# sedaprotocol/bn254

Measured on AMD Instinct MI355X. Metric: BN254 pairings/sec (batch verify), higher is better.
Workload: dtype u32

## Files before the change

bn254_amd/csrc/bn254_field.h:

```cpp
#pragma once
#include <stdint.h>

#if defined(__HIPCC__)
#include <hip/hip_runtime.h>
#define BN_DEV __device__ __forceinline__
#define BN_DEVN __device__ __noinline__
#define BN_CONST __device__ __constant__ const
#if defined(BN_INLINE_FP12_HOT)
#define BN_DEVH BN_DEV
#else
#define BN_DEVH BN_DEVN
#endif
#if defined(BN_INLINE_FE_HOT)
#define BN_DEVF BN_DEV
#else
#define BN_DEVF BN_DEVN
#endif
#if defined(__HIP_DEVICE_COMPILE__) && !defined(BN_NO_ASSUME_LDS)
#define BN_ASSUME_LDS(ptr) __builtin_assume(__builtin_amdgcn_is_shared((const void*)(ptr)))
#else
#define BN_ASSUME_LDS(ptr) do { } while (0)
#endif
#if defined(BN_INLINE_MILLER)
#define BN_DEVM BN_DEV
// ... 1052 lines not shown
  fp6_inv(d, d);
  fp6_mul<91>(t0, a.c1, d);
  fp6_mul<95>(r.c0, a.c0, d);
  fp6_neg(r.c1, t0);
}
#if defined(BN_INLINE_MUL_LINE)
BN_DEVH void fp12_mul_line(Fp12& r, const Fp12& f, const Fp2& l0, const Fp2& l1, const Fp2& l2) {
#else
BN_DEVN void fp12_mul_line(Fp12& r, const Fp12& f, const Fp2& l0, const Fp2& l1, const Fp2& l2) {
#endif
  Fp6 t0, t1, s, u;
  fp6_mul_fp2(t0, f.c0, l0);
  fp6_mul_01<110>(t1, f.c1, l1, l2);
  fp6_add(s, f.c0, f.c1); fp6_site_n<113>(s, s);
  fp6_mul_01<116>(u, s, NS(119, fp2_add(l0, l1)), l2);
  fp6_sub(u, u, t0);
  fp6_sub(u, u, t1);
  fp6_mul_v(s, t1);
  fp6_add(s, t0, s);
  fp6_site_r<120>(r.c0, s);
  fp6_site_r<123>(r.c1, u);
}
#if defined(BN_SPLIT_FP2) && defined(BN_FP6_LAZY) && !defined(BN_FP6_LAZY_ONLY_SQR)
BN_DEVH void fp12_mul_line2(Fp12& r, const Fp12& f, const Fp6& b0, const Fp2& b10, const Fp2& b11) {
  Fp6 t0, t1, s, u, bs;
  fp6_mul_lazy(t0, f.c0, b0);
  fp6_mul_01_lazy(t1, f.c1, b10, b11);
  fp6_add(s, f.c0, f.c1);
  bs.c0 = NS(306, fp2_add(b0.c0, b10)); bs.c1 = NS(307, fp2_add(b0.c1, b11)); bs.c2 = b0.c2;
  fp6_mul_lazy(u, s, bs);
  fp6_sub(u, u, t0);
  fp6_sub(u, u, t1);
  fp6_mul_v(s, t1);
  fp6_add(s, t0, s);
  fp6_site_r<308>(r.c0, s);
  fp6_site_r<311>(r.c1, u);
}
#else
BN_DEVH void fp12_mul_line2(Fp12& r, const Fp12& f, const Fp6& b0, const Fp2& b10, const Fp2& b11) {
  Fp6 t0, t1, s, u, bs;
  fp6_mul<140>(t0, f.c0, b0);
  fp6_mul_01<144>(t1, f.c1, b10, b11);
  fp6_add(s, f.c0, f.c1); fp6_site_n<147>(s, s);
  bs.c0 = NS(150, fp2_add(b0.c0, b10)); bs.c1 = NS(151, fp2_add(b0.c1, b11)); bs.c2 = b0.c2;
  fp6_mul<152>(u, s, bs);
  fp6_sub(u, u, t0);
  fp6_sub(u, u, t1);
  fp6_mul_v(s, t1);
  fp6_add(s, t0, s);
  fp6_site_r<156>(r.c0, s);
  fp6_site_r<159>(r.c1, u);
}
#endif
BN_DEV Fp2& fp12_coef(Fp12& a, int k) {
  Fp6& h = (k & 1) ? a.c1 : a.c0;
  return (k >> 1) == 0 ? h.c0 : (k >> 1) == 1 ? h.c1 : h.c2;
}
BN_DEV void fp12_frob_body(Fp12& r, const Fp12& a, int power) {
  Fp12 t = a;
  for (int k = 0; k < 6; ++k) {
    Fp2& c = fp12_coef(t, k);
    Fp2 x = (power & 1) ? fp2_conj(c) : c;
    const int32_t (*g)[BN_LIMBS] = power == 1 ? C_FROB1[k] : power == 2 ? C_FROB2[k] : C_FROB3[k];
    c = fp2_mul(x, fp2_load_const(g));
  }
  r = t;
}
BN_DEVN void fp12_frob(Fp12& r, const Fp12& a, int power) { fp12_frob_body(r, a, power); }
template <int S> BN_DEV void fp4_sqr(Fp2& r0, Fp2& r1, const Fp2& a, const Fp2& b) {
  Fp2 a2 = fp2_sqr(a), b2 = fp2_sqr(b);
  r1 = NS(S + 1, fp2_sub(fp2_sub(fp2_sqr(NS(S, fp2_add(a, b))), a2), b2));
  r0 = NS(S + 2, fp2_add(a2, fp2_mul_xi(b2)));
}
template <int S> BN_DEV void fp12_cyclotomic_sqr_body(Fp12& r, const Fp12& a) {
#if defined(BN_TRIO_DEVICE)
  const int g = trio_g3();
  Fp2 x, y, ae, ao, e, o;
#pragma unroll
  for (int i = 0; i < BN_LIMBS; ++i) {
    x.c[0].v[i] = g == 0 ? a.c0.c0.c[0].v[i] : g == 1 ? a.c1.c0.c[0].v[i] : a.c0.c1.c[0].v[i];
    y.c[0].v[i] = g == 0 ? a.c1.c1.c[0].v[i] : g == 1 ? a.c0.c2.c[0].v[i] : a.c1.c2.c[0].v[i];
    ae.c[0].v[i] = g == 0 ? a.c0.c0.c[0].v[i] : g == 1 ? a.c0.c1.c[0].v[i] : a.c0.c2.c[0].v[i];
    ao.c[0].v[i] = g == 0 ? a.c1.c1.c[0].v[i] : g == 1 ? a.c1.c2.c[0].v[i] : a.c1.c0.c[0].v[i];
  }
  fp4_sqr<S + 20>(e, o, x, y);
  const Fp2 oxi = NS(S + 9, fp2_mul_xi(o));
#pragma unroll
  for (int i = 0; i < BN_LIMBS; ++i) o.c[0].v[i] = g == 2 ? oxi.c[0].v[i] : o.c[0].v[i];
  e = fp2_lin2_reduce(e, 3, ae, -2);
  o = fp2_lin2_reduce(o, 3, ao, 2);
  const unsigned base = BN_TRIO_X6_OFF + (threadIdx.x >> 3) * BN_TRIO_X6_STRIDE, mine = base + (threadIdx.x & 7u) * (3 * BN_LIMBS);
  BN_TRIO_FENCE();
#pragma unroll
  for (int i = 0; i < BN_LIMBS; ++i) { bn_trio_lds[mine + i] = e.c[0].v[i]; bn_trio_lds[mine + BN_LIMBS + i] = o.c[0].v[i]; }
  BN_TRIO_FENCE();
  const unsigned role = threadIdx.x & 1u;
  Fp12 out;
  Fp2* dst[6] = {&out.c0.c0, &out.c1.c1, &out.c0.c1, &out.c1.c2, &out.c0.c2, &out.c1.c0};
#pragma unroll
  for (int k = 0; k < 3; ++k) {
    const unsigned from = base + (2 * k + role) * (3 * BN_LIMBS);
#pragma unroll
    for (int i = 0; i < BN_LIMBS; ++i) { dst[2 * k]->c[0].v[i] = bn_trio_lds[from + i]; dst[2 * k + 1]->c[0].v[i] = bn_trio_lds[from + BN_LIMBS + i]; }
  }
  BN_TRIO_FENCE();
  r = out;
// ... 21 lines not shown
```

bn254_amd/csrc/bn254_hip.hip:

```cpp
#include <hip/hip_runtime.h>
#include <thread>

#include <cstdio>
#include <cstdlib>
#include <cstring>
#include <new>

#include "../../include/bn254_hip.h"
#include "bn254_hash.h"
#include "bn254_io.h"
#include "bn254_pairing.h"

using namespace bn254;

#include "bn254_ws.h"
#include "bn254_lane.h"
#include "bn254_host.h"

KERNEL_SMALL void k_decode_g1(const uint8_t* pts, size_t n, uint32_t flags, Ws ws, int px, int inf_plane, int accumulate) {
  size_t i = (size_t)blockIdx.x * BN_WAVE + threadIdx.x;
  if (i >= n) return;
  G1Affine p;
  uint8_t st = decode_g1(p, pts + 64 * i, flags);
  if (st != ST_OK) g1_set_generator(p);
// ... 814 lines not shown
  if (option == BN254_OPT_TRIO_WAVE_ROLES) {
    if (value < 0 || value > 2 || (value == 2 && !c->fits_w8) || (value == 1 && !c->fits_quad)) return BN254_E_BAD_ARGUMENT;
    c->trio_wave_roles = value;
    return 0;
  }
  if (option == BN254_OPT_HASH_DIRECT_WIDTH) {
    if (value < 0 || value > 32 || (value & (value - 1))) return BN254_E_BAD_ARGUMENT;
    c->hash_direct_width = value;
    return 0;
  }
  if (option == BN254_OPT_HASH_SCHEDULE) { if (value < 0 || value > 2) return BN254_E_BAD_ARGUMENT; c->hash_schedule = value; return 0; }
  if (option == BN254_OPT_HASH_WIDE_WIDTH) { if (value < 0 || value > 64) return BN254_E_BAD_ARGUMENT; c->hash_wide_width = value; return 0; }
  if (option == BN254_OPT_HASH_TAIL_CHUNK) {
    if (value < 2 || value > 32 || (value & (value - 1))) return BN254_E_BAD_ARGUMENT;
    c->hash_tail_chunk = value;
    return 0;
  }
  if (option == BN254_OPT_NONET_MAX_BATCH) {
    HIP_TRY(hipSetDevice(c->device));
    if (value < 0 || (value > 0 && !bn254_nonet_fits_device())) return BN254_E_BAD_ARGUMENT;
    c->nonet_max_batch = value;
    return 0;
  }
  if (option == BN254_OPT_NONET_WIDE) { c->nonet_wide = value != 0; return 0; }
  if (option == BN254_OPT_LM_MAX_BATCH) {
    HIP_TRY(hipSetDevice(c->device));
    if (value < 0 || (value > 0 && !bn254_lm_fits_device())) return BN254_E_BAD_ARGUMENT;
    c->lm_max_batch = value;
    return 0;
  }
  if (option == BN254_OPT_PINNED_STAGING) { if (value < 0 || value > 16) return BN254_E_BAD_ARGUMENT; c->pinned_staging = value; return 0; }
  if (option == BN254_OPT_AGG_SORT_BY_MSG) { c->agg_sort_by_msg = value != 0; return 0; }
  if (option == BN254_OPT_AGG_T4_ROUTE) { if (value < 0 || value > 1) return BN254_E_BAD_ARGUMENT; c->agg_t4_route = value; return 0; }
  if (option == BN254_OPT_AGG_WIDE_MIN_TUPLES) { if (value < 0) return BN254_E_BAD_ARGUMENT; c->agg_wide_min_tuples = value; return 0; }
  if (option == BN254_OPT_CLOCK_PROBE) {
    HIP_TRY(hipSetDevice(c->device));
    HIP_TRY(hipDeviceSynchronize());
    if (value && !c->ws.clk) {
      HIP_TRY(hipMalloc((void**)&c->ws.clk, sizeof(unsigned long long) * 3 * BN_CLK_MAX_WG * 2));
      HIP_TRY(hipMemset(c->ws.clk, 0, sizeof(unsigned long long) * 3 * BN_CLK_MAX_WG * 2));
    } else if (!value && c->ws.clk) {
      HIP_TRY(hipFree(c->ws.clk));
      c->ws.clk = nullptr;
    }
    return 0;
  }
  if (option == BN254_OPT_HASH_MAX_TRIES) { if (value < 0 || value > 255) return BN254_E_BAD_ARGUMENT; c->hash_max_tries = value; return 0; }
  if (option == BN254_OPT_G2_FIXED_BASE) { c->g2_fixed_base = value != 0; return 0; }
  if (option == BN254_OPT_MAX_CHUNK) { if (value < 0) return BN254_E_BAD_ARGUMENT; c->max_chunk = value; return 0; }
  if (option == BN254_OPT_ASSUME_FREE_MB) { if (value < 0) return BN254_E_BAD_ARGUMENT; c->assume_free_mb = value; return 0; }
  if (option == BN254_OPT_KEY_DEDUP) { if (value < 0 || value > 1) return BN254_E_BAD_ARGUMENT; c->key_dedup = value; return 0; }
  if (option == BN254_OPT_KEY_DEDUP_MAX_KEYS) { if (value < 0 || value > KEY_DEDUP_MAX_KEYS_LIMIT) return BN254_E_BAD_ARGUMENT; c->kd_max_keys = value; return 0; }
  if (option == BN254_OPT_KEY_DEDUP_MIN_MULT) { if (value < 1) return BN254_E_BAD_ARGUMENT; c->kd_min_mult = value; return 0; }
  if (option == BN254_OPT_KEY_DEDUP_FOLD) { if (value < 0 || value > 1) return BN254_E_BAD_ARGUMENT; c->kd_fold = value; return 0; }
  if (option == BN254_OPT_KEY_DEDUP_FORCE_GENERIC) { c->kd_force_generic = value == 2 ? 2 : value != 0; return 0; }
  if (option == BN254_OPT_KEY_CACHE) { if (value < 0 || value > 1) return BN254_E_BAD_ARGUMENT; c->kd_cache = value; c->kd_cache_valid = false; return 0; }
  if (option == BN254_OPT_KEY_DEDUP_HASH_BITS) { if (value < 0 || value > 32) return BN254_E_BAD_ARGUMENT; c->kd_hash_bits = value; return 0; }
  if (option == BN254_OPT_AGGD_KEYED_ROUTE) { if (value < 0 || value > 3) return BN254_E_BAD_ARGUMENT; c->aggd_keyed_route = value; return 0; }
  if (option == BN254_OPT_AGG_RAND_MIN_PAIRS) { if (value < 0) return BN254_E_BAD_ARGUMENT; c->agg_rand_min_pairs = value; return 0; }
  if (option == BN254_OPT_AGG_RAND_GROUP_PAIRS) { if (value < 1) return BN254_E_BAD_ARGUMENT; c->agg_rand_group_pairs = value; return 0; }
  if (option == BN254_OPT_BITMAP_TABLE_MAX_KEYS) { if (value < 0) return BN254_E_BAD_ARGUMENT; c->bm_table_max_keys = value; return 0; }
  if (option == BN254_OPT_BITMAP_RAND_MIN_TUPLES) { if (value < 0) return BN254_E_BAD_ARGUMENT; c->bmr_min_tuples = value; return 0; }
  if (option == BN254_OPT_BITMAP_RAND_MAX_KEYS) { if (value < 0) return BN254_E_BAD_ARGUMENT; c->bmr_max_keys = value; return 0; }
  if (option == BN254_OPT_COLLECT_WAVE_MIN_SHARES) { if (value < 1) return BN254_E_BAD_ARGUMENT; c->collect_wave_min = value; return 0; }
  if (option == BN254_OPT_POLY_EVAL_WAVE_MIN_COEFFS) { if (value < 1) return BN254_E_BAD_ARGUMENT; c->pe_wave_min = value; return 0; }
  if (option == BN254_OPT_COLLECT_RAND_MIN_SHARES) { if (value < 0) return BN254_E_BAD_ARGUMENT; c->collect_rand_min_shares = value; return 0; }
  if (option == BN254_OPT_COLLECT_RAND_MIN_PER_KEY) { if (value < 0) return BN254_E_BAD_ARGUMENT; c->collect_rand_min_per_key = value; return 0; }
  if (option == BN254_OPT_THRESHOLD_OPT_MIN_SHARES) { if (value < 0) return BN254_E_BAD_ARGUMENT; c->th_opt_min_shares = value; return 0; }
  if (option == BN254_OPT_COLLECT_OPT_MIN_SHARES) { if (value < 0) return BN254_E_BAD_ARGUMENT; c->collect_opt_min_shares = value; return 0; }
  if (option == BN254_OPT_MERGE_WAVE_MIN_PARTS) { if (value < 1) return BN254_E_BAD_ARGUMENT; c->merge_wave_min = value; return 0; }
  if (option == BN254_OPT_MERGE_OPT_MIN_PARTS) { if (value < 0) return BN254_E_BAD_ARGUMENT; c->merge_opt_min_parts = value; return 0; }
  if (option == BN254_OPT_COLLECT_OPT_MIN_TUPLE_SHARES) { if (value < 0) return BN254_E_BAD_ARGUMENT; c->collect_opt_min_tuple_shares = value; return 0; }
  if (option == BN254_OPT_BITMAP_RAND_GROUP_TUPLES) { if (value < 1) return BN254_E_BAD_ARGUMENT; c->bmr_group_tuples = value; return 0; }
  if (option == BN254_OPT_BITMAP_ROUTE) { if (value < 0 || value > 2) return BN254_E_BAD_ARGUMENT; c->bm_route = value; return 0; }
  return BN254_E_BAD_ARGUMENT;
}
int bn254_ctx_last_clocks(bn254_ctx* c, double sclk_mhz[3]) {
  if (!c || !sclk_mhz || !c->ws.clk) return BN254_E_BAD_ARGUMENT;
  HIP_TRY(hipSetDevice(c->device));
  int wall_khz = 0;
  HIP_TRY(hipDeviceGetAttribute(&wall_khz, hipDeviceAttributeWallClockRate, c->device));
  const size_t words = (size_t)3 * BN_CLK_MAX_WG * 2;
  unsigned long long* h = (unsigned long long*)malloc(words * sizeof(unsigned long long));
  if (!h) return BN254_E_NO_MEMORY;
  hipError_t e = hipDeviceSynchronize();
  if (e == hipSuccess) e = hipMemcpy(h, c->ws.clk, words * sizeof(unsigned long long), hipMemcpyDeviceToHost);
  if (e == hipSuccess) e = hipMemset(c->ws.clk, 0, words * sizeof(unsigned long long));
  if (e != hipSuccess) { free(h); return -(int)e; }
  for (int k = 0; k < 3; ++k) {
    double cyc = 0, wall = 0;
    for (size_t w = 0; w < BN_CLK_MAX_WG; ++w) {
      const unsigned long long a = h[((size_t)k * BN_CLK_MAX_WG + w) * 2], b = h[((size_t)k * BN_CLK_MAX_WG + w) * 2 + 1];
      if (b) { cyc += (double)a; wall += (double)b; }
    }
    sclk_mhz[k] = wall > 0 ? cyc / wall * (double)wall_khz * 1e-3 : 0.0;
  }
  free(h);
  return 0;
}
int bn254_ctx_last_kernel_ms(bn254_ctx* c, float ms[4]) {
  if (!c || !ms || !c->ev_valid) return BN254_E_BAD_ARGUMENT;
  if (c->ev_layout == EV_COLLECT) {
    static const int from[4] = {1, 4, 2, 3}, to[4] = {2, 0, 3, 4};
    HIP_TRY(hipEventSynchronize(c->ev[0]));
    for (int i = 0; i < 4; ++i) HIP_TRY(hipEventElapsedTime(&ms[i], c->ev[from[i]], c->ev[to[i]]));
    return 0;
  }
  HIP_TRY(hipEventSynchronize(c->ev[4]));
  for (int i = 0; i < 4; ++i) HIP_TRY(hipEventElapsedTime(&ms[i], c->ev[i], c->ev[i + 1]));
  if (c->ev_layout == EV_HASH_FIRST) { float t = ms[0]; ms[0] = ms[1]; ms[1] = t; }
  return 0;
}


}
int launch_final_exp_layout(bn254_ctx* c, hipStream_t s, size_t n, int use_hash, uint8_t* d_status, int fe) {
  switch (fe) {
    case BN_FE_NONET_WIDE: return bn254_nonet_final_exp(n, c->ws, use_hash, d_status, s, 1);
    case BN_FE_NONET: return bn254_nonet_final_exp(n, c->ws, use_hash, d_status, s, 0);
    case BN_FE_OCTET: return bn254_trio_final_exp(n, c->ws, use_hash, d_status, s);
    default: return bn254_pair_final_exp(n, c->ws, use_hash, d_status, nullptr, nullptr, s);
  }
}
int launch_verify_miller_fe(bn254_ctx* c, hipStream_t s, size_t n, int pairs, int use_hash, uint8_t* d_status, bool mark) {
  if (!c->pair_lanes) {
    const unsigned g = grid_for(n);
    if (pairs == BN_PAIRS_CHECK_PKS) k_miller_cpk<<<g, BN_WAVE, 0, s>>>(n, c->ws);
    else k_miller_verify<<<g, BN_WAVE, 0, s>>>(n, c->ws, nullptr, nullptr);
    if (mark) PROF_MARK(3);
    k_final_exp<<<g, BN_WAVE, 0, s>>>(n, 1, 1, 1, c->ws, use_hash, nullptr, d_status, 0, 0, nullptr, nullptr);
    return 0;
  }
  const BnRoute r = route_for(c, n);
  int rc;
  switch (r.miller) {
    case BN_ML_LANE_MACHINE: rc = bn254_lm_miller_verify(n, c->ws, s, pairs); break;
    case BN_ML_WAVE_ROLES:
      rc = c->trio_wave_roles == 2 ? bn254_w8_miller_verify(n, c->ws, s, pairs)
           : c->trio_wave_roles ? bn254_quad_miller_verify(n, c->ws, s, pairs) : bn254_trio_miller_verify(n, c->ws, s, pairs);
      break;
    default: rc = bn254_pair_miller_verify(n, c->ws, nullptr, nullptr, s, pairs); break;
  }
  if (rc) return rc;
  if (mark) PROF_MARK(3);
  return launch_final_exp_layout(c, s, n, use_hash, d_status, r.fe);
}

extern "C" {
static int verify_tail(bn254_ctx* c, hipStream_t s, size_t n, uint8_t* d_status, bool split, const KeyDedup* kd, int hash_first) {
  int rc;
  if (kd) {
    HIP_TRY(hipStreamWaitEvent(s, c->kd_join, 0));
    const KeyTable kt = {kd->lines, kd->st, kd->inf, kd->max_keys};
    if (c->kd_fold) rc = bn254_pair_miller_verify_keyed_fold(n, c->ws, kd->key_idx, kt, kd->fold, s, 0, nullptr, kd->ctl + KD_CTL_KEYED_N);
    else rc = bn254_pair_miller_verify_keyed(n, c->ws, kd->key_idx, kt, s, 0, nullptr, kd->ctl + KD_CTL_KEYED_N);
    if (rc) return rc;
    if ((rc = bn254_pair_miller_verify(n, c->ws, nullptr, kd->ctl + KD_CTL_GENERIC_N, s))) return rc;
    PROF_MARK(3);
    if ((rc = bn254_pair_final_exp(n, c->ws, 1, d_status, nullptr, nullptr, s))) return rc;
    HIP_TRY(hipEventRecord(c->kd_done, s));
  } else if (split) {
    const unsigned g = grid_for(n);
    k_miller_verify_split<<<2 * g, BN_WAVE, 0, s>>>(n, c->ws.stride / 2, g, c->ws);
    PROF_MARK(3);
    k_final_exp<<<g, BN_WAVE, 0, s>>>(n, 2, 1, c->ws.stride / 2, c->ws, 1, nullptr, d_status, 0, 0, nullptr, nullptr);
  } else if ((rc = launch_verify_miller_fe(c, s, n, BN_PAIRS_VERIFY, 1, d_status, true))) return rc;
  PROF_MARK(4);
  prof_done(c, hash_first ? EV_HASH_FIRST : EV_DECODE_FIRST);
  HIP_TRY(hipGetLastError());
  return 0;
}
static int verify_after_decode(bn254_ctx* c, hipStream_t s, const uint8_t* d_msgs, const uint64_t* d_off, size_t n, uint8_t* d_status, bool split,
                               const KeyDedup* kd = nullptr) {
  PROF_MARK(1);
  if (const int rc = launch_hash_rounds(c, s, d_msgs, d_off, n, PL_P2X, BY_P2_INF, nullptr)) return rc;
  PROF_MARK(2);
  return verify_tail(c, s, n, d_status, split, kd, 0);
}

int bn254_batch_verify_device(bn254_ctx* c, const uint8_t* d_msgs, const uint64_t* d_off, const uint8_t* d_sigs, const uint8_t* d_pks,
                              size_t n, uint32_t flags, uint8_t* d_status, void* stream) {
  MsgsLenScope msgs_len_scope(c);
  if (!c || (n && (!d_msgs || !d_off || !d_sigs || !d_pks || !d_status))) return BN254_E_BAD_ARGUMENT;
  if (n == 0) return 0;
  if (misaligned(d_sigs) || misaligned(d_pks) || ((uintptr_t)d_off & 7u)) return BN254_E_MISALIGNED;
  HIP_TRY(hipSetDevice(c->device));
  bool split = c->split_miller && n <= BN_SPLIT_MAX_N;
  bool key_dedup = c->key_dedup && c->kd_max_keys > 0 && c->pair_lanes && !split && n <= 0xFFFFFFFFu &&
                         route_for(c, n).miller == BN_ML_LANE_PAIRS && route_for(c, n).fe == BN_FE_LANE_PAIRS;
  if (const size_t chunk = ws_chunk_for(c, n, split ? 2 : 1, key_dedup))
    return verify_device_sliced(n, chunk, [&](size_t lo, size_t len) {
      return bn254_batch_verify_device(c, d_msgs, d_off + lo, d_sigs + 64 * lo, d_pks + 128 * lo, len, flags, d_status + lo, stream);
    });
  int rc = ws_reserve(c, split ? 2 * n : n);
  if (rc) return rc;
  KeyDedup kd;
  if (key_dedup) {
    rc = kd_reserve(c, n, kd);
    if (rc == KD_NO_ROOM) key_dedup = false;
    else if (rc) return rc;
    rc = 0;
  }
  c->kd_last_run = key_dedup;
  hipStream_t s = stream ? (hipStream_t)stream : c->stream;
  CallDone call_done(c, s);
  PROF_MARK(0);
  if (key_dedup) {
// ... 291 lines not shown
```

bn254_amd/csrc/bn254_pair.hip:

```cpp
#include <hip/hip_runtime.h>

#define BN_SPLIT_FP2 1
#if defined(BN_PAIR_FP6_LAZY) && !defined(BN_FP6_LAZY)
#define BN_FP6_LAZY 1
#endif
#ifndef BN_PAIR_NO_SQR_DPP_ASM
#define BN_PAIR_SQR_DPP_ASM 1
#endif
#ifndef BN_PAIR_CALL_FP12_HOT
#define BN_INLINE_FP12_HOT 1
#endif
#ifndef BN_PAIR_CALL_MUL_LINE
#define BN_INLINE_MUL_LINE 1
#endif
#ifndef BN_PAIR_CALL_FE_HOT
#define BN_INLINE_FE_HOT 1
#endif
#ifndef BN_PRIO_SHIFT
#define BN_PRIO_SHIFT 1
#endif
#define BN_SET_STEP_PRIORITY(step)                                                        \
  do {                                                                                    \
    if (((step) & ((1 << BN_PRIO_SHIFT) - 1)) == 0) {                                     \
      int q_ = ((step) >> BN_PRIO_SHIFT) & 3;                                             \
// ... 156 lines not shown
  k_miller_verify_keyed_pair<<<(unsigned)((2 * n + BN_PAIR_WG - 1) / BN_PAIR_WG), BN_PAIR_WG, 0, s>>>(n, ws, key_idx, kt, base, map, count);
  HIP_TRY(hipGetLastError());
  return 0;
}
struct WsMonomials {
  int32_t* f0;
  size_t stride;
  uint32_t i;
  __device__ __forceinline__ void uniform() {
    f0 = (int32_t*)bn_wave_uniform(f0);
    stride = ((size_t)(uint32_t)__builtin_amdgcn_readfirstlane((int)(uint32_t)(stride >> 32)) << 32) | (uint32_t)__builtin_amdgcn_readfirstlane((int)(uint32_t)stride);
  }
  __device__ __forceinline__ void put(int pair, int j, const Fp& x) {
#pragma unroll
    for (int k = 0; k < BN_LIMBS; ++k) f0[((size_t)(3 * pair + j) * BN_LIMBS + k) * stride + i] = x.v[k];
  }
  __device__ __forceinline__ Fp get(int pair, int j) const {
    Fp r;
#pragma unroll
    for (int k = 0; k < BN_LIMBS; ++k) r.v[k] = f0[((size_t)(3 * pair + j) * BN_LIMBS + k) * stride + i];
    return r;
  }
};
KERNEL_PAIR void k_miller_verify_keyed_fold_pair(size_t n, Ws ws, const uint32_t* key_idx, KeyTable kt, const int32_t* fold, size_t base, const uint32_t* map,
                                                 const uint32_t* count) {
  size_t i = ((size_t)blockIdx.x * BN_PAIR_WG + threadIdx.x) >> 1;
  if (i >= n) return;
  if (count && i >= *count) return;
  if (map) i = map[i];
  uint32_t key = key_idx[i];
  i += base;
  uint8_t kst = ST_OK;
  if (key >= kt.n_keys) { kst = ST_INDEX_OOB; key = 0; }
  else kst = kt.st[key];
  const bool key_inf = kst != ST_OK || kt.inf[key] != 0;
  if ((threadIdx.x & 1u) == 0) {
    const uint8_t prev = ws_byte(ws, BY_ST_DECODE, i);
    ws_byte(ws, BY_ST_DECODE, i) = prev != ST_OK ? prev : kst;
  }
  G1Affine sig, h;
  ws_load_g1(ws, PL_P1X, BY_P1_INF, i, sig);
  ws_load_g1(ws, PL_P2X, BY_P2_INF, i, h);
  __shared__ Fp12PairSlot lds_f[BN_PAIR_WG];
  Fp12& f = lds_f[threadIdx.x].v;
  const WsMonomials mono = {ws.planes + (size_t)PL_F0 * BN_LIMBS * ws.stride, ws.stride, (uint32_t)i};
  BN_CLK_BEGIN(ws);
  miller_loop_keyed_fold<true>(f, h, key_inf, kt.lines, fold, key, sig, mono);
  BN_CLK_END(ws, 0);
  ws_store_f12_own(ws, i, f);
}
int bn254_pair_miller_verify_keyed_fold(size_t n, Ws ws, const uint32_t* key_idx, KeyTable kt, const int32_t* fold, hipStream_t s, size_t base,
                                        const uint32_t* map, const uint32_t* count) {
  k_miller_verify_keyed_fold_pair<<<(unsigned)((2 * n + BN_PAIR_WG - 1) / BN_PAIR_WG), BN_PAIR_WG, 0, s>>>(n, ws, key_idx, kt, fold, base, map, count);
  HIP_TRY(hipGetLastError());
  return 0;
}
KERNEL_PAIR void k_miller_var_pair(size_t n, Ws ws) {
  size_t i = ((size_t)blockIdx.x * BN_PAIR_WG + threadIdx.x) >> 1;
  if (i >= n) return;
  G1Affine p;
  G2Affine q;
  ws_load_g1(ws, PL_P1X, BY_P1_INF, i, p);
  q.x = ws_load_fp2_own(ws, PL_QX0, i);
  q.y = ws_load_fp2_own(ws, PL_QY0, i);
  q.inf = ws_byte(ws, BY_Q_INF, i) != 0;
  __shared__ Fp12PairSlot lds_f[BN_PAIR_WG];
  Fp12& f = lds_f[threadIdx.x].v;
  miller_loop<true, false, true>(f, p, q, p);
  ws_store_f12_own(ws, i, f);
}
template <int ITEMS_PER_PAIR>
__device__ __forceinline__ void miller_rand_pair_body(size_t n, size_t n_groups, Ws ws, size_t gbase) {
  constexpr unsigned PAIRS_PER_GROUP = BN_WAVE / ITEMS_PER_PAIR;
  constexpr unsigned GROUPS_PER_WG = (BN_PAIR_WG / 2) / PAIRS_PER_GROUP;
  const unsigned pair = threadIdx.x >> 1, gp = pair / PAIRS_PER_GROUP, tp = pair % PAIRS_PER_GROUP;
  const size_t group = (size_t)blockIdx.x * GROUPS_PER_WG + gp;
  const size_t i0 = group * BN_WAVE + (size_t)tp * ITEMS_PER_PAIR;
  __shared__ Fp12PairSlot lds_f[BN_PAIR_WG];
  Fp12& f = lds_f[threadIdx.x].v;
  G1Affine a0;
  G2Affine pk0;
  const size_t j0 = i0 < n ? i0 : n - 1;
  ws_load_g1(ws, PL_HASHX, BY_A_INF, j0, a0);
  if (i0 >= n) a0.inf = true;
  pk0.x = ws_load_fp2_own(ws, PL_QX0, j0); pk0.y = ws_load_fp2_own(ws, PL_QY0, j0); pk0.inf = ws_byte(ws, BY_Q_INF, j0) != 0;
  if constexpr (ITEMS_PER_PAIR == 2) {
    G1Affine a1;
    G2Affine pk1;
    const size_t i1 = i0 + 1, j1 = i1 < n ? i1 : n - 1;
    ws_load_g1(ws, PL_HASHX, BY_A_INF, j1, a1);
    if (i1 >= n) a1.inf = true;
    pk1.x = ws_load_fp2_own(ws, PL_QX0, j1); pk1.y = ws_load_fp2_own(ws, PL_QY0, j1); pk1.inf = ws_byte(ws, BY_Q_INF, j1) != 0;
    miller_loop_2var<true>(f, a0, pk0, a1, pk1);
  } else {
    miller_loop<true, false, true>(f, a0, pk0, a0);
  }
  __syncthreads();
  for (unsigned stride = PAIRS_PER_GROUP / 2; stride >= 1; stride >>= 1) {
    if (tp < stride) fp12_mul(f, f, lds_f[threadIdx.x + 2 * stride].v);
    __syncthreads();
  }
  if (tp == 0 && group < n_groups) ws_store_f12_own(ws, gbase + group, f);
}
KERNEL_PAIR void k_miller_rand_pair(size_t n, size_t n_groups, Ws ws, size_t gbase) { miller_rand_pair_body<1>(n, n_groups, ws, gbase); }
KERNEL_PAIR void k_miller_rand2_pair(size_t n, size_t n_groups, Ws ws, size_t gbase) { miller_rand_pair_body<2>(n, n_groups, ws, gbase); }
KERNEL_PAIR void k_rand_tail_pair(size_t n_groups, Ws ws, size_t gbase) {
// ... 521 lines not shown
```

bn254_amd/csrc/bn254_pairing.h:

```cpp
#pragma once
#include "bn254_curve.h"


namespace bn254 {

struct G2Proj { Fp2 x, y, z; };
struct LineCoef { Fp2 c0, c1, c2; };

BN_DEVN void dbl_step(G2Proj& t, LineCoef& l) {
  Fp2 xy = fp2_mul(t.x, t.y), b = fp2_sqr(t.y), c = fp2_sqr(t.z);
  Fp2 e = fp2_mul(c, fp2_load_const(C_TWIST_3B));
  Fp2 f = fp2_add(fp2_dbl(e), e);
  Fp2 h = fp2_sub(fp2_sub(fp2_sqr(NS(200, fp2_add(t.y, t.z))), b), c);
  Fp2 x2 = fp2_sqr(t.x);
  Fp2 e2x4 = NS(201, fp2_dbl(fp2_dbl(fp2_sqr(e))));
  Fp2 e2x12 = fp2_add(fp2_dbl(e2x4), e2x4);
  G2Proj o;
  o.x = NS(203, fp2_mul(fp2_dbl(xy), NS(202, fp2_sub(b, f))));
  o.y = NS(205, fp2_sub(fp2_sqr(NS(204, fp2_add(b, f))), e2x12));
  o.z = NS(206, fp2_dbl(fp2_dbl(fp2_mul(b, h))));
  l.c0 = h;
  l.c1 = fp2_neg(fp2_add(fp2_dbl(x2), x2));
  l.c2 = fp2_sub(b, e);
  t = o;
// ... 205 lines not shown
  if (any_skip) {
    const Fp2 zero = fp2_zero();
    L.b0.c0 = fp2_select(skip, fp2_one(), L.b0.c0);
    L.b0.c1 = fp2_select(skip, zero, L.b0.c1);
    L.b0.c2 = fp2_select(skip, zero, L.b0.c2);
    L.b10 = fp2_select(skip, zero, L.b10);
    L.b11 = fp2_select(skip, zero, L.b11);
  }
}
template <class T> BN_DEV const T* bn_wave_uniform(const T* p) {
#if defined(__HIP_DEVICE_COMPILE__)
  const uint64_t v = (uint64_t)p;
  return (const T*)(((uint64_t)(uint32_t)__builtin_amdgcn_readfirstlane((int)(uint32_t)(v >> 32)) << 32) | (uint32_t)__builtin_amdgcn_readfirstlane((int)(uint32_t)v));
#else
  return p;
#endif
}
template <bool F_LDS = false, class Mono>
BN_DEVM void miller_loop_keyed_fold(Fp12& f, const G1Affine& pa, bool key_inf, const int32_t* lines, const int32_t* folds, uint32_t key, const G1Affine& pb,
                                    Mono mono) {
  if constexpr (F_LDS) BN_ASSUME_LDS(&f);
  fp12_set_one(f);
  lines = bn_wave_uniform(lines); folds = bn_wave_uniform(folds);
  mono.uniform();
  typedef const int32_t (*LinePtr)[2][2][BN_LIMBS];
  typedef const int32_t (*FoldPtr)[5][2][BN_LIMBS];
  const bool skip_a = pa.inf || key_inf, skip_b = pb.inf;
#if defined(__HIPCC__)
  const bool any_skip = __builtin_amdgcn_ballot_w64(skip_a || skip_b) != 0;
#else
  const bool any_skip = skip_a || skip_b;
#endif
  g1_monomials_put(mono, 0, pa);
  g1_monomials_put(mono, 1, pb);
  const LinePtr tab = (LinePtr)(lines + (size_t)key * (BN_N_FIXED_LINES * 2 * 2 * BN_LIMBS));
  const FoldPtr fold = (FoldPtr)(folds + (size_t)key * (BN_N_FOLD_ROWS * 5 * 2 * BN_LIMBS));
  auto folded_a = [&](int r) { LineProduct L; folded_row_product<286>(L, fold[r], pa, mono, 0, skip_a, any_skip); fp12_mul_line2(f, f, L.b0, L.b10, L.b11); };
  auto folded_b = [&](int r) { LineProduct L; folded_row_product<287>(L, C_NEG_G2_FOLD[r], pb, mono, 1, skip_b, any_skip); fp12_mul_line2(f, f, L.b0, L.b10, L.b11); };
  int idx = 0, r = 0;
  for (int d = 0; d < 64; ++d) {
    BN_SET_STEP_PRIORITY(d);
    fp12_sqr(f, f);
    const bool digit = C_ATE_NAF[d] != 0;
    if (digit) folded_b(r);
    if (!digit) {
      KeyLine la;
      la.c0 = fp2_load_const(tab[idx][0]); la.c1 = fp2_load_const(tab[idx][1]);
      mul_by_two_table_lines(f, la, pa.x, pa.y, skip_a, idx, pb.x, pb.y, skip_b, any_skip);
      ++idx;
    } else { folded_a(r); ++r; idx += 2; }
  }
  folded_b(r);
  folded_a(r);
}
#endif
BN_DEV void mul_by_two_key_lines(Fp12& f, const KeyLine& la, const Fp& pax, const Fp& pay, bool skip_a, const KeyLine& lb, const Fp& pbx, const Fp& pby,
                                 bool skip_b, bool any_skip) {
  const Fp2 l0 = fp2_mul_fp(la.c0, pay), l1 = fp2_mul_fp(la.c1, pax);
  const Fp2 m0 = fp2_mul_fp(lb.c0, pby), m1 = fp2_mul_fp(lb.c1, pbx);
  const Fp2 v0 = fp2_mul(l0, m0), v1 = fp2_mul(l1, m1);
  const Fp2 x01 = fp2_sub(fp2_sub(fp2_mul(NS(280, fp2_add(l0, l1)), NS(281, fp2_add(m0, m1))), v0), v1);
  Fp6 b0;
  b0.c0 = NS(282, fp2_add(v0, fp2_load_const(C_XI_MONT))); b0.c1 = v1; b0.c2 = NS(283, fp2_add(l1, m1));
  Fp2 b10 = NS(284, x01), b11 = NS(285, fp2_add(l0, m0));
  if (any_skip) {
    const Fp2 one = fp2_one(), zero = fp2_zero();
    const bool both = skip_a && skip_b, only_a = skip_a && !skip_b, only_b = skip_b && !skip_a;
    b0.c0 = fp2_select(both, one, fp2_select(only_a, m0, fp2_select(only_b, l0, b0.c0)));
    b0.c1 = fp2_select(skip_a || skip_b, zero, b0.c1);
    b0.c2 = fp2_select(skip_a || skip_b, zero, b0.c2);
    b10 = fp2_select(both, zero, fp2_select(only_a, m1, fp2_select(only_b, l1, b10)));
    b11 = fp2_select(both, zero, fp2_select(skip_a || skip_b, one, b11));
  }
  fp12_mul_line2(f, f, b0, b10, b11);
}
template <int W, bool F_LDS = false>
BN_DEVM void miller_loop_tables(Fp12& f, const G1Affine& pa, bool skip_a, const int32_t (*taba)[2][2][BN_LIMBS], const G1Affine& pb, bool skip_b,
                                const int32_t (*tabb)[2][2][BN_LIMBS]) {
  static_assert(W == 1 || W == 2, "one or two table pairs per lane pair");
  if constexpr (F_LDS) BN_ASSUME_LDS(&f);
  fp12_set_one(f);
#if defined(__HIPCC__)
  const bool any_skip = __builtin_amdgcn_ballot_w64(skip_a || (W == 2 && skip_b)) != 0;
#else
  const bool any_skip = skip_a || (W == 2 && skip_b);
#endif
  int idx = 0;
  auto step = [&]() {
    if constexpr (W == 2) {
      KeyLine la, lb;
      la.c0 = fp2_load_const(taba[idx][0]); la.c1 = fp2_load_const(taba[idx][1]);
      lb.c0 = fp2_load_const(tabb[idx][0]); lb.c1 = fp2_load_const(tabb[idx][1]);
      mul_by_two_key_lines(f, la, pa.x, pa.y, skip_a, lb, pb.x, pb.y, skip_b, any_skip);
    } else {
      LineCoef l;
      l.c0 = fp2_load_const(taba[idx][0]); l.c1 = fp2_load_const(taba[idx][1]); l.c2 = fp2_one();
      mul_by_line(f, l, pa.x, pa.y, skip_a);
    }
    ++idx;
  };
  for (int d = 0; d < 64; ++d) {
    BN_SET_STEP_PRIORITY(d);
    fp12_sqr(f, f);
    step();
    if (C_ATE_NAF[d] != 0) step();
  }
// ... 752 lines not shown
```

bn254_amd/csrc/bn254_ws.h:

```cpp
#pragma once
#include <stddef.h>

#define BN_WAVE 64
#define BN_SPLIT_MAX_N ((size_t)98304)
#define TRIO_MAX_BATCH_DEFAULT 16384
#define NONET_WIDE_MAX_BATCH 1024
#define NONET_MAX_BATCH_DEFAULT 3072
#define LM_MAX_BATCH_DEFAULT 1536
enum BnMillerLayout { BN_ML_LANE_MACHINE = 0, BN_ML_WAVE_ROLES = 1, BN_ML_LANE_PAIRS = 2 };
enum BnFeLayout { BN_FE_NONET_WIDE = 0, BN_FE_NONET = 1, BN_FE_OCTET = 2, BN_FE_LANE_PAIRS = 3 };
struct BnRouteLimits { size_t lm_max, nonet_wide_max, nonet_max, small_max; };
struct BnRoute { int miller, fe; };
static inline BnRoute bn_route(const BnRouteLimits& L, size_t n) {
  BnRoute r = {BN_ML_LANE_PAIRS, BN_FE_LANE_PAIRS};
  if (n > L.small_max) return r;
  r.miller = n <= L.lm_max ? BN_ML_LANE_MACHINE : BN_ML_WAVE_ROLES;
  r.fe = n <= L.nonet_max ? (n <= L.nonet_wide_max ? BN_FE_NONET_WIDE : BN_FE_NONET) : BN_FE_OCTET;
  return r;
}
static inline int bn_route_table(const BnRouteLimits& L, size_t* max_n, BnRoute* route, int cap) {
  size_t b[4] = {L.lm_max, L.nonet_wide_max, L.nonet_max, L.small_max};
  for (int i = 0; i < 4; ++i) if (b[i] > L.small_max) b[i] = L.small_max;
  for (int i = 0; i < 4; ++i) for (int j = i + 1; j < 4; ++j) if (b[j] < b[i]) { size_t t = b[i]; b[i] = b[j]; b[j] = t; }
  int rows = 0;
// ... 101 lines not shown
  return r;
}
__device__ __forceinline__ void pool_store_fp(const Pool& p, int e, size_t j, const Fp& a) {
  int32_t* w = p.planes + pool_word(p, e, j);
#pragma unroll
  for (int k = 0; k < BN_LIMBS; ++k) w[k] = a.v[k];
}
#define HIP_TRY(expr)                                      \
  do {                                                     \
    hipError_t e_ = (expr);                                \
    if (e_ != hipSuccess) return -(int)e_;                 \
  } while (0)

__attribute__((visibility("hidden"))) int bn254_pair_miller_verify(size_t n, Ws ws, const uint32_t* map, const uint32_t* count, hipStream_t s,
                                                                   int mode = 0);
__attribute__((visibility("hidden"))) int bn254_pair_miller_var(size_t n, Ws ws, hipStream_t s);
__attribute__((visibility("hidden"))) int bn254_pair_leaf_floor(size_t n, Ws ws, hipStream_t s, int mode);
__attribute__((visibility("hidden"))) int bn254_pair_fe_program(size_t n, Ws ws, const unsigned char* prog, hipStream_t s);
__attribute__((visibility("hidden"))) int bn254_pair_final_exp_product(size_t n, size_t k, Ws ws, uint8_t* gt_out, uint8_t* status_out, int raw_only,
                                                                       hipStream_t s);
__attribute__((visibility("hidden"))) int bn254_pair_final_exp(size_t n, Ws ws, int use_hash, uint8_t* status_out, const uint32_t* map,
                                                               const uint32_t* count, hipStream_t s, size_t base = 0);
__attribute__((visibility("hidden"))) int bn254_pair_miller_rand(size_t n, size_t n_groups, int items_per_pair, Ws ws, size_t gbase, hipStream_t s);
__attribute__((visibility("hidden"))) int bn254_pair_rand_tail(size_t n_groups, Ws ws, size_t gbase, hipStream_t s);
struct AggdSlots { const uint32_t* slot_agg; const uint64_t* incl; const uint64_t* lo; const uint64_t* hi; };
__attribute__((visibility("hidden"))) int bn254_pair_aggd_miller(size_t n_slots, Ws ws, AggdSlots sl, size_t gbase, size_t pbase, uint32_t* pseg, int last,
                                                                 hipStream_t s);
__attribute__((visibility("hidden"))) int bn254_pair_aggd_level(size_t n_elems, Ws ws, const uint32_t* seg, size_t ebase, size_t gbase, size_t pbase,
                                                                 uint32_t* pseg, int last, hipStream_t s);
__attribute__((visibility("hidden"))) int bn254_pair_aggd_tail(size_t n, Ws ws, size_t gbase, size_t obase, hipStream_t s);
__attribute__((visibility("hidden"))) int bn254_pair_aggregate(const uint32_t* tuple_msg, const uint64_t* tuple_off, const uint32_t* signer_idx, size_t n,
                                                               size_t n_signers, size_t n_msgs, Pool pk_pool, Pool sig_pool, Pool h_pool, Pool sub_pool,
                                                               size_t n_groups, Pool sub1_pool, size_t groups4, Ws ws, hipStream_t s,
                                                               const uint32_t* perm = nullptr, const Pool* wide2_pool = nullptr,
                                                               const Pool* wide1_pool = nullptr);
__attribute__((visibility("hidden"))) int bn254_pair_g2_mul_fixed(const uint8_t* d_scalars, size_t n, int reduce, Pool comb, uint8_t* d_out, uint8_t* d_status,
                                                                  hipStream_t s);
#define BN_G2_COMB_RECORDS (65 * 8 + 1)
__attribute__((visibility("hidden"))) int bn254_pair_g1_mul_fixed(const uint8_t* d_scalars, size_t n, int reduce, Pool comb, uint8_t* d_out, uint8_t* d_status,
                                                                  hipStream_t s);
#define BN_G1_COMB_RECORDS (65 * 8 + 3)
__attribute__((visibility("hidden"))) int bn254_pair_decode_g2(const uint8_t* pts, size_t n, uint32_t flags, Ws ws, int accumulate, hipStream_t s);
__attribute__((visibility("hidden"))) int bn254_pair_decompress_g2(const uint8_t* in, size_t n, Ws ws, hipStream_t s, int skip_subgroup_test = 0);

#define BN_KEY_LINE_WORDS (2 * 2 * BN_LIMBS)
struct KeyTable { const int32_t* lines; const uint8_t* st; const uint8_t* inf; uint32_t n_keys; };
__attribute__((visibility("hidden"))) int bn254_lm_miller_verify_keyed(size_t n, Ws ws, const uint32_t* key_idx, KeyTable kt, hipStream_t s);
__attribute__((visibility("hidden"))) int bn254_pair_miller_verify_keyed(size_t n, Ws ws, const uint32_t* key_idx, KeyTable kt, hipStream_t s, size_t base = 0,
                                                                         const uint32_t* map = nullptr, const uint32_t* count = nullptr);
#define BN_KEY_FOLD_WORDS (5 * 2 * BN_LIMBS)
__attribute__((visibility("hidden"))) int bn254_pair_miller_verify_keyed_fold(size_t n, Ws ws, const uint32_t* key_idx, KeyTable kt, const int32_t* fold,
                                                                              hipStream_t s, size_t base = 0, const uint32_t* map = nullptr,
                                                                              const uint32_t* count = nullptr);
#define AGGD_KEYED_W1_MAX_SLOTS 65536
__attribute__((visibility("hidden"))) int bn254_pair_aggd_keyed(size_t n_slots, int width, Ws ws, AggdSlots sl, const uint32_t* key_idx, KeyTable kt,
                                                                size_t gbase, size_t pbase, uint32_t* pseg, int last, hipStream_t s);
__attribute__((visibility("hidden"))) int bn254_pair_aggd_move(size_t n, Ws ws, size_t gbase, hipStream_t s);
#define AGG_RAND_MIN_PAIRS_DEFAULT 65536
#define AGG_RAND_GROUP_PAIRS_DEFAULT 1024
#define AGGR_SUM_WG 256
#define AGGR_PART_WORDS (3 * BN_LIMBS)
struct AggrScale { const uint32_t* pair_agg; const uint32_t* key_idx; const uint8_t* key_inf; const uint64_t* lo; uint32_t* nagg; uint32_t* ebkt;
                   uint64_t* cnt; uint64_t G; uint32_t n_keys; };
struct AggrSum { const uint32_t* perm; const uint64_t* tp; uint32_t* bkey; size_t m, gbase, cbase, tbase; uint32_t n_keys; };
__attribute__((visibility("hidden"))) int bn254_aggr_scale(size_t m, size_t n, Ws ws, size_t gbase, AggrScale a, const uint32_t* seed_be, int mode,
                                                           hipStream_t s);
__attribute__((visibility("hidden"))) int bn254_aggr_scatter(size_t n_entries, const uint32_t* ebkt, uint64_t* start, uint32_t* perm, uint32_t* eseg,
                                                             size_t n_b, uint32_t n_keys, const uint64_t* cnt, uint64_t* tp, hipStream_t s);
__attribute__((visibility("hidden"))) int bn254_aggr_glimits(size_t n_groups, uint32_t n_keys, size_t tbase, const uint64_t* cnt, const uint64_t* tp,
                                                             uint64_t* glo, uint64_t* ghi, Ws ws, size_t cbase, hipStream_t s);
__attribute__((visibility("hidden"))) int bn254_aggr_sum(size_t n_elems, int level0, Ws ws, AggrSum a, const uint32_t* seg_in, const int32_t* part_in,
                                                         uint32_t* pseg_out, int32_t* part_out, int last, hipStream_t s);
__attribute__((visibility("hidden"))) int bn254_aggr_collect(size_t n, Ws ws, size_t gbase, const uint64_t* lo, uint64_t G, const uint32_t* nagg,
                                                             const uint8_t* gst, uint8_t* status, uint8_t* queued, size_t n_groups, const uint64_t* glo,
                                                             const uint64_t* ghi, uint32_t* stats, hipStream_t s);
__attribute__((visibility("hidden"))) int bn254_pair_aggd_keyed_queued(size_t n_slots, int width, Ws ws, AggdSlots sl, const uint32_t* key_idx, KeyTable kt,
                                                                       size_t gbase, size_t pbase, uint32_t* pseg, int last, const uint8_t* queued,
                                                                       hipStream_t s);

#define BITMAP_TABLE_MAX_KEYS_DEFAULT 4096
struct BmKeysArg { const int32_t* xy; const uint8_t* st; const uint8_t* inf; const uint32_t* bad; uint32_t n_keys; };
__attribute__((visibility("hidden"))) int bn254_pair_bitmap_sum(const uint32_t* d_bits, size_t bm_words, size_t n, BmKeysArg keys, const int32_t* rec,
                                                                const uint8_t* rec_inf, Ws ws, hipStream_t s);

#define BITMAP_RAND_MIN_TUPLES_DEFAULT 81920
#define BITMAP_RAND_MAX_KEYS_DEFAULT 256
#define BITMAP_RAND_GROUP_TUPLES_DEFAULT 4096
#define COLLECT_WAVE_MIN_SHARES_DEFAULT 16
#define POLY_EVAL_WAVE_MIN_COEFFS_DEFAULT 16
#define COLLECT_RAND_MIN_SHARES_DEFAULT 65664
#define COLLECT_RAND_MIN_PER_KEY_DEFAULT 42
#define COLLECT_OPT_MIN_SHARES_DEFAULT 1539
#define COLLECT_OPT_MIN_TUPLE_SHARES_DEFAULT 1
#define MERGE_WAVE_MIN_PARTS_DEFAULT 16
#define THRESHOLD_OPT_MIN_SHARES_DEFAULT 513
#define MERGE_OPT_MIN_PARTS_DEFAULT 64
__attribute__((visibility("hidden"))) int bn254_aggd_scan_add(hipStream_t s, const uint64_t* in, size_t n, uint64_t* out, uint64_t* tot);
__attribute__((visibility("hidden"))) int bn254_aggd_scan_max(hipStream_t s, const uint64_t* in, size_t n, uint64_t* out, uint64_t* tot);
__attribute__((visibility("hidden"))) int bn254_aggd_keyed_slot_map(hipStream_t s, size_t n, const uint64_t* lo, const uint64_t* hi, int width,
                                                                    uint64_t* kincl, uint64_t* tot, size_t n_slots, uint32_t* slot_agg);

#define KEY_DEDUP_MAX_KEYS_DEFAULT 1024
#define KEY_DEDUP_MIN_MULT_DEFAULT 16
#define KEY_DEDUP_FOLD_DEFAULT 1
#define KEY_DEDUP_MAX_KEYS_LIMIT 16384
#define KD_MAX_PROBES 64u
#define KD_EMPTY 0xFFFFFFFFu
enum { KD_OVERFLOW = 1, KD_DEGENERATE = 2 };
enum { KD_CTL_D = 0, KD_CTL_FLAGS, KD_CTL_KEYED_N, KD_CTL_GENERIC_N, KD_CTL_BUILD, KD_CTL_HITS, KD_CTL_DROPPED, KD_CTL_WORDS = 8 };
enum { KD_DROP_CAPACITY = 1, KD_DROP_RESET = 2 };
struct KeyDedup {
  uint32_t* table;
  uint32_t* slot_id;
  uint32_t* slot_of;
  uint32_t* key_idx;
  uint32_t* rep;
  uint32_t* ctl;
  int32_t* lines;
  int32_t* c2;
  int32_t* fold;
  uint8_t* st;
  uint8_t* inf;
  uint32_t* row_of;
  uint32_t* build_row;
  uint32_t* build_rep;
  uint32_t* c_keys;
  uint32_t* c_index;
  uint32_t* c_state;
  uint32_t slot_mask, hash_mask, max_keys, min_mult, index_mask;
};
__attribute__((visibility("hidden"))) int bn254_kd_enqueue(const uint8_t* d_pks, size_t n, uint32_t flags, KeyDedup kd, int force_generic, int cache_reset,
                                                           int cache_on, hipStream_t s);
#define KD_BYTES_PER_ITEM ((size_t)(2 * 4 + 2) * sizeof(uint32_t))
#define KD_FOLD_KEY_WORDS (BN_N_FOLD_ROWS * BN_KEY_FOLD_WORDS)
static_assert(KD_FOLD_KEY_WORDS >= BN_N_FIXED_LINES * 2 * BN_LIMBS, "a key's raw c2 fits where its folded rows go");
#define KD_BYTES_PER_KEY ((size_t)(BN_N_FIXED_LINES * BN_KEY_LINE_WORDS + KD_FOLD_KEY_WORDS) * sizeof(int32_t) + (4 + 32 + 4) * sizeof(uint32_t) + 2)

__attribute__((visibility("hidden"))) int bn254_trio_miller_verify(size_t n, Ws ws, hipStream_t s, int mode = 0);
__attribute__((visibility("hidden"))) int bn254_quad_miller_verify(size_t n, Ws ws, hipStream_t s, int mode = 0);
__attribute__((visibility("hidden"))) int bn254_w8_miller_verify(size_t n, Ws ws, hipStream_t s, int mode = 0);
__attribute__((visibility("hidden"))) bool bn254_trio_fits_device();
__attribute__((visibility("hidden"))) bool bn254_quad_fits_device(int eight_waves);
__attribute__((visibility("hidden"))) int bn254_trio_final_exp(size_t n, Ws ws, int use_hash, uint8_t* status_out, hipStream_t s);
__attribute__((visibility("hidden"))) bool bn254_lm_fits_device();
__attribute__((visibility("hidden"))) int bn254_lm_miller_verify(size_t n, Ws ws, hipStream_t s, int mode = 0);
__attribute__((visibility("hidden"))) int bn254_lm_g2_subgroup(size_t n, Ws ws, hipStream_t s, int fail_status = 4 );
__attribute__((visibility("hidden"))) bool bn254_nonet_fits_device();
__attribute__((visibility("hidden"))) int bn254_nonet_final_exp(size_t n, Ws ws, int use_hash, uint8_t* status_out, hipStream_t s, int wide = 0);
__attribute__((visibility("hidden"))) int bn254_nonet_final_exp_product(size_t n, size_t k, Ws ws, uint8_t* gt_out, uint8_t* status_out, hipStream_t s);
#endif
```

Before: 15.85 million.

## Add unit-normalized keyed Miller loop with sparse line multiplication as default fold

Adds a keyed Miller loop variant that multiplies each precomputed table line separately, with the line normalized to a unit leading coefficient. This lets each line multiply use cheap Fp6-by-Fp2 products in place of the fuller line-pair multiply. The variant becomes the default key-dedup mode. It trades the previous folded two-line product for two sparser multiplies per step, so whether it helps depends on the relative cost of those paths.

```diff
diff --git a/bn254_amd/csrc/bn254_field.h b/bn254_amd/csrc/bn254_field.h
--- a/bn254_amd/csrc/bn254_field.h
+++ b/bn254_amd/csrc/bn254_field.h
@@ -1128,6 +1128,27 @@
   fp6_site_r<159>(r.c1, u);
 }
 #endif
+BN_DEVH void fp12_mul_unit_line(Fp12& r, const Fp12& f, const Fp2& l0, const Fp2& l1, bool skip = false, bool any_skip = false) {
+  Fp6 t0, p1, t1, s, u;
+  fp6_mul_fp2(t0, f.c0, l0);
+  fp6_mul_fp2(p1, f.c1, l1);
+  fp6_add(s, f.c0, f.c1);
+  fp6_mul_fp2(u, s, fp2_add(l0, l1));
+  fp6_sub(u, u, t0);
+  fp6_sub(u, u, p1);
+  fp6_mul_v(s, f.c0);
+  fp6_add(u, u, s);
+  fp6_mul_v(t1, f.c1);
+  fp6_add(t1, p1, t1);
+  fp6_mul_v(s, t1);
+  fp6_add(s, t0, s);
+  if (any_skip) {
+    s.c0 = fp2_select(skip, f.c0.c0, s.c0); s.c1 = fp2_select(skip, f.c0.c1, s.c1); s.c2 = fp2_select(skip, f.c0.c2, s.c2);
+    u.c0 = fp2_select(skip, f.c1.c0, u.c0); u.c1 = fp2_select(skip, f.c1.c1, u.c1); u.c2 = fp2_select(skip, f.c1.c2, u.c2);
+  }
+  fp6_site_r<450>(r.c0, s);
+  r.c1.c0 = NS(453, u.c0); r.c1.c1 = NR(454, u.c1); r.c1.c2 = NR(455, u.c2);
+}
 BN_DEV Fp2& fp12_coef(Fp12& a, int k) {
   Fp6& h = (k & 1) ? a.c1 : a.c0;
   return (k >> 1) == 0 ? h.c0 : (k >> 1) == 1 ? h.c1 : h.c2;
diff --git a/bn254_amd/csrc/bn254_hip.hip b/bn254_amd/csrc/bn254_hip.hip
--- a/bn254_amd/csrc/bn254_hip.hip
+++ b/bn254_amd/csrc/bn254_hip.hip
@@ -890,7 +890,7 @@
   if (option == BN254_OPT_KEY_DEDUP) { if (value < 0 || value > 1) return BN254_E_BAD_ARGUMENT; c->key_dedup = value; return 0; }
   if (option == BN254_OPT_KEY_DEDUP_MAX_KEYS) { if (value < 0 || value > KEY_DEDUP_MAX_KEYS_LIMIT) return BN254_E_BAD_ARGUMENT; c->kd_max_keys = value; return 0; }
   if (option == BN254_OPT_KEY_DEDUP_MIN_MULT) { if (value < 1) return BN254_E_BAD_ARGUMENT; c->kd_min_mult = value; return 0; }
-  if (option == BN254_OPT_KEY_DEDUP_FOLD) { if (value < 0 || value > 1) return BN254_E_BAD_ARGUMENT; c->kd_fold = value; return 0; }
+  if (option == BN254_OPT_KEY_DEDUP_FOLD) { if (value < 0 || value > 2) return BN254_E_BAD_ARGUMENT; c->kd_fold = value; return 0; }
   if (option == BN254_OPT_KEY_DEDUP_FORCE_GENERIC) { c->kd_force_generic = value == 2 ? 2 : value != 0; return 0; }
   if (option == BN254_OPT_KEY_CACHE) { if (value < 0 || value > 1) return BN254_E_BAD_ARGUMENT; c->kd_cache = value; c->kd_cache_valid = false; return 0; }
   if (option == BN254_OPT_KEY_DEDUP_HASH_BITS) { if (value < 0 || value > 32) return BN254_E_BAD_ARGUMENT; c->kd_hash_bits = value; return 0; }
@@ -990,7 +990,8 @@
   if (kd) {
     HIP_TRY(hipStreamWaitEvent(s, c->kd_join, 0));
     const KeyTable kt = {kd->lines, kd->st, kd->inf, kd->max_keys};
-    if (c->kd_fold) rc = bn254_pair_miller_verify_keyed_fold(n, c->ws, kd->key_idx, kt, kd->fold, s, 0, nullptr, kd->ctl + KD_CTL_KEYED_N);
+    if (c->kd_fold == 2) rc = bn254_pair_miller_verify_keyed_unit(n, c->ws, kd->key_idx, kt, s, 0, nullptr, kd->ctl + KD_CTL_KEYED_N);
+    else if (c->kd_fold) rc = bn254_pair_miller_verify_keyed_fold(n, c->ws, kd->key_idx, kt, kd->fold, s, 0, nullptr, kd->ctl + KD_CTL_KEYED_N);
     else rc = bn254_pair_miller_verify_keyed(n, c->ws, kd->key_idx, kt, s, 0, nullptr, kd->ctl + KD_CTL_KEYED_N);
     if (rc) return rc;
     if ((rc = bn254_pair_miller_verify(n, c->ws, nullptr, kd->ctl + KD_CTL_GENERIC_N, s))) return rc;
diff --git a/bn254_amd/csrc/bn254_pair.hip b/bn254_amd/csrc/bn254_pair.hip
--- a/bn254_amd/csrc/bn254_pair.hip
+++ b/bn254_amd/csrc/bn254_pair.hip
@@ -232,6 +232,38 @@
 int bn254_pair_miller_verify_keyed_fold(size_t n, Ws ws, const uint32_t* key_idx, KeyTable kt, const int32_t* fold, hipStream_t s, size_t base,
                                         const uint32_t* map, const uint32_t* count) {
   k_miller_verify_keyed_fold_pair<<<(unsigned)((2 * n + BN_PAIR_WG - 1) / BN_PAIR_WG), BN_PAIR_WG, 0, s>>>(n, ws, key_idx, kt, fold, base, map, count);
+  HIP_TRY(hipGetLastError());
+  return 0;
+}
+KERNEL_PAIR void k_miller_verify_keyed_unit_pair(size_t n, Ws ws, const uint32_t* key_idx, KeyTable kt, size_t base, const uint32_t* map,
+                                                 const uint32_t* count) {
+  size_t i = ((size_t)blockIdx.x * BN_PAIR_WG + threadIdx.x) >> 1;
+  if (i >= n) return;
+  if (count && i >= *count) return;
+  if (map) i = map[i];
+  uint32_t key = key_idx[i];
+  i += base;
+  uint8_t kst = ST_OK;
+  if (key >= kt.n_keys) { kst = ST_INDEX_OOB; key = 0; }
+  else kst = kt.st[key];
+  const bool key_inf = kst != ST_OK || kt.inf[key] != 0;
+  if ((threadIdx.x & 1u) == 0) {
+    const uint8_t prev = ws_byte(ws, BY_ST_DECODE, i);
+    ws_byte(ws, BY_ST_DECODE, i) = prev != ST_OK ? prev : kst;
+  }
+  G1Affine sig, h;
+  ws_load_g1(ws, PL_P1X, BY_P1_INF, i, sig);
+  ws_load_g1(ws, PL_P2X, BY_P2_INF, i, h);
+  __shared__ Fp12PairSlot lds_f[BN_PAIR_WG];
+  Fp12& f = lds_f[threadIdx.x].v;
+  BN_CLK_BEGIN(ws);
+  miller_loop_keyed_unit<true>(f, h, key_inf, kt.lines, key, sig);
+  BN_CLK_END(ws, 0);
+  ws_store_f12_own(ws, i, f);
+}
+int bn254_pair_miller_verify_keyed_unit(size_t n, Ws ws, const uint32_t* key_idx, KeyTable kt, hipStream_t s, size_t base, const uint32_t* map,
+                                        const uint32_t* count) {
+  k_miller_verify_keyed_unit_pair<<<(unsigned)((2 * n + BN_PAIR_WG - 1) / BN_PAIR_WG), BN_PAIR_WG, 0, s>>>(n, ws, key_idx, kt, base, map, count);
   HIP_TRY(hipGetLastError());
   return 0;
 }
diff --git a/bn254_amd/csrc/bn254_pairing.h b/bn254_amd/csrc/bn254_pairing.h
--- a/bn254_amd/csrc/bn254_pairing.h
+++ b/bn254_amd/csrc/bn254_pairing.h
@@ -281,6 +281,66 @@
   }
   folded_b(r);
   folded_a(r);
+}
+BN_DEV void mul_by_unit_table_line(Fp12& f, const Fp2& c0, const Fp2& c1, const Fp& px, const Fp& py, bool skip, bool any_skip) {
+  const Fp2 l0 = fp2_mul_fp(c0, py), l1 = fp2_mul_fp(c1, px);
+  fp12_mul_unit_line(f, f, l0, l1, skip, any_skip);
+}
+BN_DEV void set_two_table_lines(Fp12& f, const KeyLine& la, const Fp& pax, const Fp& pay, bool skip_a, int idx, const Fp& pbx, const Fp& pby,
+                                bool skip_b, bool any_skip) {
+  const Fp2 l0 = fp2_mul_fp(la.c0, pay), l1 = fp2_mul_fp(la.c1, pax);
+  const Fp2 m0 = fp2_mul_fp(fp2_load_const(C_NEG_G2_LINES[idx][0]), pby), m1 = fp2_mul_fp(fp2_load_const(C_NEG_G2_LINES[idx][1]), pbx);
+  const Fp2 v0 = fp2_mul(l0, m0), v1 = fp2_mul(l1, m1);
+  const Fp2 x01 = fp2_sub(fp2_sub(fp2_mul(NS(460, fp2_add(l0, l1)), NS(461, fp2_add(m0, m1))), v0), v1);
+  Fp6 b0;
+  b0.c0 = NS(462, fp2_add(v0, fp2_load_const(C_XI_MONT))); b0.c1 = v1; b0.c2 = NS(463, fp2_add(l1, m1));
+  Fp2 b10 = NS(464, x01), b11 = NS(465, fp2_add(l0, m0));
+  if (any_skip) {
+    const Fp2 one = fp2_one(), zero = fp2_zero();
+    const bool both = skip_a && skip_b, only_a = skip_a && !skip_b, only_b = skip_b && !skip_a;
+    b0.c0 = fp2_select(both, one, fp2_select(only_a, m0, fp2_select(only_b, l0, b0.c0)));
+    b0.c1 = fp2_select(skip_a || skip_b, zero, b0.c1);
+    b0.c2 = fp2_select(skip_a || skip_b, zero, b0.c2);
+    b10 = fp2_select(both, zero, fp2_select(only_a, m1, fp2_select(only_b, l1, b10)));
+    b11 = fp2_select(both, zero, fp2_select(skip_a || skip_b, one, b11));
+  }
+  f.c0 = b0;
+  f.c1.c0 = b10; f.c1.c1 = b11; f.c1.c2 = fp2_zero();
+}
+template <bool F_LDS = false>
+BN_DEVM void miller_loop_keyed_unit(Fp12& f, const G1Affine& pa, bool key_inf, const int32_t* lines, uint32_t key, const G1Affine& pb) {
+  if constexpr (F_LDS) BN_ASSUME_LDS(&f);
+  lines = bn_wave_uniform(lines);
+  typedef const int32_t (*LinePtr)[2][2][BN_LIMBS];
+  const bool skip_a = pa.inf || key_inf, skip_b = pb.inf;
+#if defined(__HIPCC__)
+  const bool any_skip = __builtin_amdgcn_ballot_w64(skip_a || skip_b) != 0;
+#else
+  const bool any_skip = skip_a || skip_b;
+#endif
+  const LinePtr tab = (LinePtr)(lines + (size_t)key * (BN_N_FIXED_LINES * 2 * 2 * BN_LIMBS));
+  int idx = 0;
+  auto pair = [&]() {
+    mul_by_unit_table_line(f, fp2_load_const(C_NEG_G2_LINES[idx][0]), fp2_load_const(C_NEG_G2_LINES[idx][1]), pb.x, pb.y, skip_b, any_skip);
+    mul_by_unit_table_line(f, fp2_load_const(tab[idx][0]), fp2_load_const(tab[idx][1]), pa.x, pa.y, skip_a, any_skip);
+    ++idx;
+  };
+  {
+    BN_SET_STEP_PRIORITY(0);
+    KeyLine la;
+    la.c0 = fp2_load_const(tab[0][0]); la.c1 = fp2_load_const(tab[0][1]);
+    set_two_table_lines(f, la, pa.x, pa.y, skip_a, 0, pb.x, pb.y, skip_b, any_skip);
+    ++idx;
+    if (C_ATE_NAF[0] != 0) pair();
+  }
+  for (int d = 1; d < 64; ++d) {
+    BN_SET_STEP_PRIORITY(d);
+    fp12_sqr(f, f);
+    pair();
+    if (C_ATE_NAF[d] != 0) pair();
+  }
+  pair();
+  pair();
 }
 #endif
 BN_DEV void mul_by_two_key_lines(Fp12& f, const KeyLine& la, const Fp& pax, const Fp& pay, bool skip_a, const KeyLine& lb, const Fp& pbx, const Fp& pby,
diff --git a/bn254_amd/csrc/bn254_ws.h b/bn254_amd/csrc/bn254_ws.h
--- a/bn254_amd/csrc/bn254_ws.h
+++ b/bn254_amd/csrc/bn254_ws.h
@@ -177,6 +177,8 @@
 __attribute__((visibility("hidden"))) int bn254_pair_miller_verify_keyed_fold(size_t n, Ws ws, const uint32_t* key_idx, KeyTable kt, const int32_t* fold,
                                                                               hipStream_t s, size_t base = 0, const uint32_t* map = nullptr,
                                                                               const uint32_t* count = nullptr);
+__attribute__((visibility("hidden"))) int bn254_pair_miller_verify_keyed_unit(size_t n, Ws ws, const uint32_t* key_idx, KeyTable kt, hipStream_t s, size_t base = 0,
+                                                                              const uint32_t* map = nullptr, const uint32_t* count = nullptr);
 #define AGGD_KEYED_W1_MAX_SLOTS 65536
 __attribute__((visibility("hidden"))) int bn254_pair_aggd_keyed(size_t n_slots, int width, Ws ws, AggdSlots sl, const uint32_t* key_idx, KeyTable kt,
                                                                 size_t gbase, size_t pbase, uint32_t* pseg, int last, hipStream_t s);
@@ -227,7 +229,7 @@
 
 #define KEY_DEDUP_MAX_KEYS_DEFAULT 1024
 #define KEY_DEDUP_MIN_MULT_DEFAULT 16
-#define KEY_DEDUP_FOLD_DEFAULT 1
+#define KEY_DEDUP_FOLD_DEFAULT 2
 #define KEY_DEDUP_MAX_KEYS_LIMIT 16384
 #define KD_MAX_PROBES 64u
 #define KD_EMPTY 0xFFFFFFFFu
```

New measurement: 16.38 million, median of 6. +3.4%, better.
